# cvg/diffmvs

Measured on AMD Instinct MI355X. Metric: depth-maps/sec (640x512, 5 src views), higher is better.
Workload: dtype f32

## Files before the change

diffmvs_amd/_lib.py:

```python
from __future__ import annotations

import ctypes as C
import os

PKG = os.path.dirname(os.path.abspath(__file__))
HIP_LIB_PATH = os.environ.get("DMVS_LIB") or os.path.join(PKG, "libdmvs_hip.so")

ACT_NONE, ACT_RELU, ACT_SIGMOID, ACT_TANH, ACT_SILU = range(5)
IN_PLAIN, IN_UPSAMPLE2, IN_UNSHUFFLE2, IN_ZEROINSERT2 = range(4)
LAYOUT_NCHW, LAYOUT_NHWC, LAYOUT_NHWC_BF16, LAYOUT_NHWC_F16 = 0, 1, 2, 3
DTYPE_F32, DTYPE_BF16, DTYPE_F16, DTYPE_F32_PLAIN = 0, 1, 2, 3
ARITH_F32, ARITH_BF16, ARITH_SPLIT = 0, 1, 2
EW_DEPTH_TO_DISP, EW_DISP_TO_DEPTH = 0, 1

_P = C.c_void_p
_I = C.c_int32
_F = C.c_float


class Conv2dDesc(C.Structure):
    _fields_ = [
        ("in0", _P), ("in1", _P), ("mul0", _P), ("weight", _P), ("scale", _P), ("shift", _P),
        ("residual", _P), ("gru_z", _P), ("gru_h", _P), ("out", _P), ("gn_stats", _P), ("out_mul", _P),
        ("B", _I), ("c0", _I), ("c1", _I), ("Hin", _I), ("Win", _I), ("Hout", _I), ("Wout", _I),
# ... 18 lines not shown
        ("ref", _P), ("src", _P), ("rt", _P), ("inv_depth", _P), ("confidence", _P), ("view_w", _P),
        ("disp_min", _P), ("disp_max", _P), ("out_cost", _P), ("out_samples", _P), ("worklist", _P),
        ("B", _I), ("S", _I), ("C", _I), ("G", _I), ("n", _I), ("H", _I), ("W", _I), ("vw_shift", _I),
        ("cost_cstride", _I), ("cost_coffset", _I), ("samp_cstride", _I), ("samp_coffset", _I),
        ("interval", _F), ("min_radius", _F), ("max_radius", _F), ("feat_dtype", _I), ("tune", _I),
    ]


SIGNATURES = {
    "dmvs_abi_version": [],
    "dmvs_conv2d_f32": [C.POINTER(Conv2dDesc), _P],
    "dmvs_featurenet_stem_f32": [_P, _P, _P, _P, _P, _P, _P, _P, _I, _I, _I, _I, _P],
    "dmvs_featurenet_stem3_f32": [_P, _P, _P, _P, _P, _P, _P, _P, _P, _P, _P, _I, _I, _I, _I, _P],
    "dmvs_featurenet_conv1_pair_f32": [_P, _P, _P, _P, _P, _P, _P, _P, _I, _I, _I, _I, _P],
    "dmvs_featurenet_fpn_tail_f32": [_P, _P, _P, _P, _P, _P, _I, _I, _I, _I, _P],
    "dmvs_conv2d_wgrad_workspace_f32": [C.POINTER(Conv2dDesc), C.POINTER(C.c_int64)],
    "dmvs_conv2d_wgrad_f32": [C.POINTER(Conv2dDesc), _P, _P, _P, _P, C.c_int64, _P],
    "dmvs_conv3d_f32": [C.POINTER(Conv3dDesc), _P],
    "dmvs_conv3d_wgrad_workspace_f32": [C.POINTER(Conv3dDesc), C.POINTER(C.c_int64)],
    "dmvs_conv3d_wgrad_f32": [C.POINTER(Conv3dDesc), _P, _P, _P, _P, C.c_int64, _P],
    "dmvs_compose_proj_f32": [_P, _P, _I, _I, _P],
    "dmvs_warp_volume_f32": [_P, _P, _P, _P, _I, _I, _I, _I, _I, _I, _I, _P],
    "dmvs_getcost_quad_f32": [C.POINTER(GetCostDesc), _P],
    "dmvs_warp_corr_init_quad_f32": [_P, _P, _P, _P, _P, _P, _I, _I, _I, _I, _I, _I, _I, _I, _I, _I, _I, _P],
    "dmvs_warp_corr_init_bwd_f32": [_P, _P, _P, _P, _P, _P, _P, _P, _I, _I, _I, _I, _I, _I, _I, _I, _I, _I, _P],
    "dmvs_getcost_bwd_f32": [C.POINTER(GetCostDesc), _P, _P, _P, _P],
    "dmvs_view_aggregate_bwd_f32": [_P, _P, _P, _P, _P, _P, _I, _I, _I, _I, _P],
    "dmvs_view_aggregate_f32": [_P, _P, _P, _I, _I, _I, _I, _P],
    "dmvs_sigmoid_max_d_f32": [_P, _P, _I, _I, _I, _P],
    "dmvs_depth_regress_f32": [_P, _P, _P, _P, _P, _P, _I, _I, _I, _P],
# ... 38 lines not shown
VIEW_SELECT_MAX_IMAGES, VIEW_SELECT_MAX_LIST = 16384, 1 << 23
CLOUD_MAX_RINGS, CLOUD_MAX_KEY_BITS, CLOUD_MAX_THRESHOLDS = 1024, 62, 16
CLOUD_MOMENTS, CLOUD_MAX_POLYGON = 20, 256
DEPTH_MAX_THRESHOLDS, DEPTH_SLOTS = 8, 7
SPLAT_VIEW_CHUNK, SPLAT_VIEW_DOUBLES, SPLAT_SLOTS, SPLAT_MAX_RADIUS, SPLAT_NO_PRETEST = 8, 15, 4, 16, 0x1
NORMAL_MAX_RADIUS, NORMAL_CAM_DOUBLES, NORMAL_VIEW_CHUNK, NORMAL_SLOTS = 4, 27, 8, 4
TSDF_VIEW_CHUNK, TSDF_VIEW_DOUBLES, TSDF_MAX_VIEWS, TSDF_MAX_QUADS, TSDF_NO_CULL = 8, 12, 65535, 357913941, 0x1
RASTER_VIEW_DOUBLES, RASTER_SLOTS, RASTER_SMALL, RASTER_CULL_NEG, RASTER_CULL_POS = 22, 8, 64, 0x1, 0x2
ABI_VERSION = 4
TUNE_NO_WALK, TUNE_PIECES4, TUNE_NO_LEAN, TUNE_1X1_TILED, TUNE_NO_TALL, TUNE_TALL = 0x4, 0x8, 0x100, 0x200, 0x400, 0x800
TUNE3D_PIECES4, TUNE3D_S2_DIRECT, TUNE3D_NO_PAIR = 0x1, 0x2, 0x4
TUNE_SWEEP_GLOBAL = 0x1
TUNE_WGRAD_ACCUMULATE = 0x1000
TUNE_SPLIT_ALL = 0x20000
TUNE_STEM_EXACT = 0x40000


def tune_xcd_group(n: int) -> int:
    return (int(n) & 7) << 14


def tune3d_xcd_group(n: int) -> int:
    return (int(n) & 7) << 4
TUNE_BWD_INTERLEAVED, BWD_GATHER_INTERLEAVED = 0x1, 2


def tune_tile_wx(n: int) -> int:
    return n & 3


# ... 39 lines not shown
```

diffmvs_amd/csrc/conv1_pair.hip:

```cpp

#include "dmvs_common.h"
#include "dmvs_ring.h"
#include "dmvs_lds_poison.h"

namespace {

typedef float f32x4 __attribute__((ext_vector_type(4)));
typedef uint32_t u32x4s __attribute__((ext_vector_type(4)));

constexpr int PB = 512;
constexpr int US = 80, UR = 64;
constexpr int NP = US + 4;
typedef dmvs_ring<2, NP> Ring;
constexpr int PLQ = Ring::PLQ, RINGQ = Ring::RINGQ;
constexpr int NLOAD = 2 * 2 * NP;
constexpr int SW = US + 8;
constexpr int STAGEF = 2 * 16 * SW;
constexpr int NPIECE = STAGEF / 4;


__global__ void __launch_bounds__(PB) __attribute__((amdgpu_waves_per_eu(4, 4)))
featurenet_conv1_pair_kernel(const float* __restrict__ x, const u32x4s* __restrict__ ws1, const float* __restrict__ scale1,
                             const float* __restrict__ shift1, const u32x4s* __restrict__ ws2, const float* __restrict__ scale2,
                             const float* __restrict__ shift2, float* __restrict__ y, int N, int H, int W, int nsx, int nsy) {
    __shared__ __attribute__((aligned(16))) float lds[2 * RINGQ * 4 + STAGEF];
    DMVS_LDS_POISON(lds);

    const int tid = threadIdx.x, lane = tid & 63, wave = __builtin_amdgcn_readfirstlane(tid >> 6);
    const int m = lane & 15, kq = lane >> 4;
    const int role = wave >> 2, wr = wave & 3;
    const long plane = (long)H * W;
    const int iplane = H * W;
    const int nunits = nsx * nsy * N;

    const u32x4s* const wsp = role ? ws2 : ws1;
    u32x4s wq[2][3][3];
#pragma unroll
    for (int c = 0; c < 2; ++c)
#pragma unroll
        for (int g = 0; g < 3; ++g)
#pragma unroll
            for (int pl = 0; pl < 3; ++pl) wq[c][g][pl] = wsp[(((c * 3 + g) * 3 + pl) * 4 + kq) * 16 + m];
    const float* const scp = role ? scale2 : scale1;
    const float* const shp = role ? shift2 : shift1;
    const float sc = scp ? scp[m] : 1.0f, sh = shp ? shp[m] : 0.0f;
    int taps = 0;
#pragma unroll
    for (int g = 0; g < 3; ++g) taps |= dmvs_tap_slot<3, 3, 2>(g, kq) << (4 * g);
    const u32x4s* const src = reinterpret_cast<const u32x4s*>(lds) + role * RINGQ;
    u32x4s* const in_q = reinterpret_cast<u32x4s*>(lds);
    uint16_t* const mid_h = reinterpret_cast<uint16_t*>(lds) + RINGQ * 8;
    float* const stage = lds + 2 * RINGQ * 4;
    const int pmax = role ? US - 1 : US + 1;

    const int tb = tid - PB / 2;
    int lm = m, ltb = tb;

    for (int unit = blockIdx.x; unit < nunits; unit += gridDim.x) {
        const dmvs_unit u(unit, nsx, nsy, US, UR, H);
        const int n = u.n, X0 = u.X0, Y0 = u.Y0, Yend = u.Yend;
        const int nsteps = ((Yend - Y0 + 2) >> 1) + 4;
        const float* const xb = x + (long)n * 16 * plane;
        float* const yb = y + (long)n * 16 * plane;
        const int row_lo = role ? Y0 : max(Y0 - 1, 0), row_hi = role ? Yend : min(Yend + 1, H - 1);
        const int wlim = min(US, W - X0) + (role ? 0 : 2);
        auto conv_group = [&](int row, int cg) -> f32x4 {
            const int p = min(cg * 16 + lm, pmax);
            bf16x8 ph[2], pm, pl;
            auto qp_of = [&](int s) { return Ring::operand(s, taps, row, p); };
            {
                const int qp = qp_of(0);
                pl = __builtin_bit_cast(bf16x8, src[2 * PLQ + qp]);
                ph[0] = __builtin_bit_cast(bf16x8, src[qp]);
                pm = __builtin_bit_cast(bf16x8, src[PLQ + qp]);
            }
            f32x4 a = {0.0f, 0.0f, 0.0f, 0.0f};
// ... 125 lines not shown
                }
                DMVS_LDS_BARRIER();
            }
        }
    }
}

}

extern "C" int dmvs_featurenet_conv1_pair_f32(const float* x, const void* wsplit1, const float* scale1, const float* shift1, const void* wsplit2,
                                              const float* scale2, const float* shift2, float* y, int32_t N, int32_t H, int32_t W, int32_t tune,
                                              void* stream) {
    if (!x || !wsplit1 || !wsplit2 || !y || N <= 0 || H <= 0 || W <= 0) return DMVS_EINVAL;
    if ((long)16 * H * W >= (1L << 31)) return DMVS_EINVAL;
    if ((W & 3) || (((uintptr_t)x | (uintptr_t)y | (uintptr_t)wsplit1 | (uintptr_t)wsplit2) & 15)) return DMVS_EINVAL;
    const int nsx = (W + US - 1) / US, nsy = (H + UR - 1) / UR;
    const long nunits = (long)nsx * nsy * N;
    if (nunits >= (1L << 31)) return DMVS_EINVAL;
    static const int resident = dmvs_resident_workgroups(reinterpret_cast<const void*>(featurenet_conv1_pair_kernel), PB);
    hipLaunchKernelGGL(featurenet_conv1_pair_kernel, dim3(dmvs_persistent_grid(tune, resident, nunits)), dim3(PB), 0, (hipStream_t)stream, x,
                       reinterpret_cast<const u32x4s*>(wsplit1), scale1, shift1, reinterpret_cast<const u32x4s*>(wsplit2), scale2, shift2, y, N, H, W,
                       nsx, nsy);
    return dmvs_launch_status();
}
```

diffmvs_amd/csrc/dmvs_ring.h:

```cpp
#pragma once
#include "dmvs_bf16.h"

struct dmvs_unit {
    int sx, sy, n, X0, Y0, Yend;
    __device__ __forceinline__ dmvs_unit(int unit, int nsx, int nsy, int US, int UR, int H) {
        sx = unit % nsx;
        const int uq = unit / nsx;
        sy = uq % nsy;
        n = uq / nsy;
        X0 = US * sx;
        Y0 = UR * sy;
        Yend = min(Y0 + UR, H) - 1;
    }
};

template <int KH, int KW, int SH = 4> __device__ __forceinline__ int dmvs_tap_slot(int g, int kq) {
    const int t = min(4 * g + kq, KH * KW - 1);
    return (t / KW) | ((t % KW) << SH);
}

template <int NCH, int NP> struct dmvs_ring {
    static constexpr int SLOTS = 4;
    static constexpr int PLQ = SLOTS * NCH * NP;
    static constexpr int RINGQ = 3 * PLQ;
    static __device__ __forceinline__ int slot(int row) { return (row + 4) & 3; }
    static __device__ __forceinline__ int index(int row, int chunk, int pos) { return (slot(row) * NCH + chunk) * NP + pos; }
    static __device__ __forceinline__ int operand(int s, int taps, int row, int pos) {
        const int c = s / 3, g = s - c * 3;
        const int tg = taps >> (4 * g);
// ... 29 lines not shown
```

diffmvs_amd/csrc/fpn_tail.hip:

```cpp

#include "dmvs_common.h"
#include "dmvs_ring.h"
#include "dmvs_lds_poison.h"

namespace {

typedef float f32x4 __attribute__((ext_vector_type(4)));
typedef uint32_t u32x4s __attribute__((ext_vector_type(4)));

constexpr int PB = 256;
constexpr int US = 32, UR = 64;
constexpr int NP = US + 2;
constexpr int NCH = 8;
typedef dmvs_ring<NCH, NP> Ring;
constexpr int PLQ = Ring::PLQ, RINGQ = Ring::RINGQ;
constexpr int SW = US + 8;
constexpr int C2PIECE = 2 * 32 * SW / 4;
constexpr int CW = US / 2 + 8;
constexpr int C3PIECE = 64 * CW / 4;
constexpr int LDSF = RINGQ * 4 + C2PIECE * 4 + 2 * C3PIECE * 4;
constexpr int NSTEP = NCH * 3;

__global__ void __launch_bounds__(PB) __attribute__((amdgpu_waves_per_eu(2, 2)))
featurenet_fpn_tail_kernel(const float* __restrict__ c2, const float* __restrict__ c3, const float* __restrict__ w1, const float* __restrict__ b1,
                           const u32x4s* __restrict__ ws2, float* __restrict__ y, int N, int H, int W, int nsx, int nsy) {
    __shared__ __attribute__((aligned(16))) float lds[LDSF];
    DMVS_LDS_POISON(lds);

    const int tid = threadIdx.x, lane = tid & 63, wave = __builtin_amdgcn_readfirstlane(tid >> 6);
    const int m = lane & 15, kq = lane >> 4;
    const int H2 = H >> 1, W2 = W >> 1;
    const int iplane = H * W, iplane3 = H2 * W2;
    const int nunits = nsx * nsy * N;

    float w1r[8], b1r[4];
#pragma unroll
    for (int c = 0; c < 8; ++c) w1r[c] = w1[(4 * c + kq) * 64 + 16 * wave + m];
#pragma unroll
    for (int r = 0; r < 4; ++r) b1r[r] = b1 ? b1[16 * wave + 4 * kq + r] : 0.0f;
    const int nt = wave & 1, rr = wave >> 1;
    unsigned lwb = (unsigned)(kq * 32 + nt * 16 + m) * 16u;
    auto wload = [&](int sp) -> u32x4s {
        return *reinterpret_cast<const u32x4s*>(reinterpret_cast<const char*>(ws2 + sp * 128) + lwb);
    };
    int taps = 0;
#pragma unroll
    for (int g = 0; g < 3; ++g) taps |= dmvs_tap_slot<3, 3, 2>(g, kq) << (4 * g);
    u32x4s* const ring = reinterpret_cast<u32x4s*>(lds);
    float* const st2 = lds + RINGQ * 4;
    float* const st3 = st2 + C2PIECE * 4;

    int lm = m, ltid = tid;

    for (int unit = blockIdx.x; unit < nunits; unit += gridDim.x) {
        const dmvs_unit u(unit, nsx, nsy, US, UR, H);
        const int n = u.n, X0 = u.X0, Y0 = u.Y0, Yend = u.Yend;
        const int Q = (Yend - Y0 + 1) >> 1;
        const float* const c2b = c2 + (long)n * 32 * iplane;
        const float* const c3b = c3 + (long)n * 64 * iplane3;
        float* const yb = y + (long)n * 32 * iplane;

        auto stage_c3 = [&](int row3, int lt) {
#pragma unroll
            for (int k = 0; k < 2; ++k) {
                if (k * PB + wave * 64 < C3PIECE) {
                    const int e = k * PB + lt;
                    const int ch = e / (CW / 4), pc = e - ch * (CW / 4);
                    const int col = (X0 >> 1) - 4 + 4 * pc;
                    const bool ok = row3 >= 0 && row3 < H2 && col >= 0 && col < W2;
                    const float* srcp = ok ? c3b + (ch * iplane3 + row3 * W2 + col) : dmvs_zero16;
                    float* dstp = st3 + (((row3 + 2) & 1) * C3PIECE + k * PB + wave * 64) * 4;
                    __builtin_amdgcn_global_load_lds(srcp, DMVS_LDS_PTR(dstp), 16, 0, 0);
// ... 101 lines not shown
    }
}

}

extern "C" int dmvs_featurenet_fpn_tail_f32(const float* c2, const float* c3, const float* w_inner, const float* b_inner, const void* wsplit_out,
                                            float* y, int32_t N, int32_t H, int32_t W, int32_t tune, void* stream) {
    if (!c2 || !c3 || !w_inner || !wsplit_out || !y || N <= 0 || H <= 0 || W <= 0) return DMVS_EINVAL;
    if ((H & 1) || (W & 7) || (long)64 * H * W >= (1L << 31)) return DMVS_EINVAL;
    if ((((uintptr_t)c2 | (uintptr_t)c3 | (uintptr_t)y | (uintptr_t)wsplit_out) & 15) || ((uintptr_t)w_inner & 3) || ((uintptr_t)b_inner & 3))
        return DMVS_EINVAL;
    const int nsx = (W + US - 1) / US, nsy = (H + UR - 1) / UR;
    const long nunits = (long)nsx * nsy * N;
    if (nunits >= (1L << 31)) return DMVS_EINVAL;
    static const int resident = dmvs_resident_workgroups(reinterpret_cast<const void*>(featurenet_fpn_tail_kernel), PB);
    hipLaunchKernelGGL(featurenet_fpn_tail_kernel, dim3(dmvs_persistent_grid(tune, resident, nunits)), dim3(PB), 0, (hipStream_t)stream, c2, c3, w_inner, b_inner,
                       reinterpret_cast<const u32x4s*>(wsplit_out), y, N, H, W, nsx, nsy);
    return dmvs_launch_status();
}
```

diffmvs_amd/csrc/stem3.hip:

```cpp

#include "dmvs_common.h"
#include "dmvs_ring.h"
#include "dmvs_lds_poison.h"

#include <type_traits>

namespace {

typedef float f32x4 __attribute__((ext_vector_type(4)));
typedef uint32_t u32x4s __attribute__((ext_vector_type(4)));

constexpr int UC = 32, UR = 32;
constexpr int INW = 72;
constexpr int INROW = 3 * INW, INGRP = 4 * INROW;
constexpr int INSLOTS = 3;
constexpr int INF = INSLOTS * INGRP;
constexpr int NPIECE = INGRP / 4;
constexpr int MW = 2 * UC + 5, CW = 2 * UC + 3;
constexpr int MPL = 8 * MW, CPL = 8 * CW;
constexpr int MIDF = 3 * MPL * 4, C0F = 3 * CPL * 4;
constexpr int K0S = 9;
constexpr int K2S = 7;

__global__ void __launch_bounds__(DMVS_BLOCK) __attribute__((amdgpu_waves_per_eu(2, 2)))
featurenet_stem3_kernel(const float* __restrict__ x, const float* __restrict__ w0, const float* __restrict__ scale0, const float* __restrict__ shift0,
                        const float* __restrict__ w1, const float* __restrict__ scale1, const float* __restrict__ shift1,
                        const float* __restrict__ w2, const float* __restrict__ scale2, const float* __restrict__ shift2, float* __restrict__ y,
                        int N, int H, int W, int nsx, int nsy) {
    __shared__ __attribute__((aligned(16))) float lds[INF + MIDF + C0F];
    DMVS_LDS_POISON(lds);
    float* const s_in = lds;
    float* const s_mid = lds + INF;
    float* const s_c0 = s_mid + MIDF;

    const int tid = threadIdx.x, lane = tid & 63, wave = __builtin_amdgcn_readfirstlane(tid >> 6);
    const int m = lane & 15, kq = lane >> 4;
    const int Ho = H >> 1, Wo = W >> 1;
    const long plane = (long)H * W, oplane = (long)Ho * Wo;
    const int nunits = nsx * nsy * N;

    float a0[K0S];
    int koff[K0S];
#pragma unroll
    for (int s = 0; s < K0S; ++s) {
        const int k = 4 * s + kq;
        const int ci = k / 12, j = (k - ci * 12) / 3, kx = k % 3;
        const int ky = m < 8 ? j : j - 1;
        a0[s] = (ky >= 0 && ky <= 2) ? w0[(ci * 9 + ky * 3 + kx) * 8 + (m & 7)] : 0.0f;
        const int koff_a = j * INROW + ci * INW + kx;
        koff[s] = koff_a | ((koff_a + (j >= 2 ? 0 : 4 * INSLOTS * INROW)) << 16);
    }
    float sc0[4], sh0[4], sc1[4], sh1[4];
#pragma unroll
    for (int r = 0; r < 4; ++r) {
// ... 12 lines not shown
    int off2[K2S];
#pragma unroll
    for (int s = 0; s < K2S; ++s) {
        const int sl = 4 * s + kq;
        float wv[8];
#pragma unroll
        for (int ci = 0; ci < 8; ++ci) wv[ci] = sl < 25 ? w2[(ci * 25 + sl) * 16 + m] : 0.0f;
        dmvs_split3_bf16x8(wv, w2h[s], w2m[s], w2l[s]);
        off2[s] = dmvs_tap_slot<5, 5>(s, kq);
    }
    const float sc2 = scale2 ? scale2[m] : 1.0f, sh2 = shift2 ? shift2[m] : 0.0f;
    const bool vec = (Wo & 3) == 0 && ((uintptr_t)y & 15) == 0;

    const int p_i = tid / (NPIECE / 4), p_rem = tid - p_i * (NPIECE / 4);
    const int p_ci = p_rem / (INW / 4), p_c = (p_rem - p_ci * (INW / 4)) * 4;
    auto stage = [&](int unit, int kg, int slot) {
        const dmvs_unit u(unit, nsx, nsy, UC, UR, Ho);
        const int row = 2 * u.Y0 - 5 + 4 * kg + p_i, col = 2 * u.X0 - 4 + p_c;
        if (tid < NPIECE) {
            const bool ok = row >= 0 && row < H && col >= 0 && col < W;
            const float* srcp = ok ? x + ((long)u.n * 3 + p_ci) * plane + (long)row * W + col : dmvs_zero16;
            float* dstp = s_in + slot * INGRP + wave * 256;
            __builtin_amdgcn_global_load_lds(srcp, DMVS_LDS_PTR(dstp), 16, 0, 0);
        }
    };

    auto steps_of = [&](int unit) {
        const dmvs_unit u(unit, nsx, nsy, UC, UR, Ho);
        return ((u.Yend - u.Y0 + 2) >> 1) + 2;
    };
    int s_unit = blockIdx.x, s_k = 0, s_slot = 0, s_steps = s_unit < nunits ? steps_of(s_unit) : 0;
    auto stage_next = [&]() {
        if (s_unit < nunits) {
            stage(s_unit, s_k, s_slot);
            s_slot = s_slot == INSLOTS - 1 ? 0 : s_slot + 1;
            if (++s_k == s_steps) {
                s_unit += gridDim.x;
                s_k = 0;
                s_steps = s_unit < nunits ? steps_of(s_unit) : 0;
            }
        }
    };
    int islot = 0, pslot = INSLOTS - 1;
    int unit = blockIdx.x;
    stage_next();
    stage_next();
    DMVS_DMA_BARRIER();
    for (; unit < nunits; unit += gridDim.x) {
        const dmvs_unit u(unit, nsx, nsy, UC, UR, Ho);
        const int n = u.n, ox0 = u.X0, oy0 = u.Y0, X0 = 2 * ox0, Y0 = 2 * oy0;
        const int nsteps = steps_of(unit);
        for (int k = 0; k < nsteps; ++k, pslot = islot, islot = islot == INSLOTS - 1 ? 0 : islot + 1) {
            {
                const int sbeg = k == 0 ? MW : 0;
                const int ng = (2 * MW - sbeg + 15) >> 4;
                auto conv00 = [&](auto ngc, int g0) {
                    constexpr int NG = decltype(ngc)::value;
                    int q[NG], pm[NG];
                    float b[NG][K0S];
                    f32x4 acc[NG];
#pragma unroll
                    for (int i = 0; i < NG; ++i) {
                        const int p = min(sbeg + (g0 + 4 * i) * 16 + m, 2 * MW - 1);
                        q[i] = p >= MW ? 1 : 0;
                        pm[i] = p - q[i] * MW;
                        const int rb = q[i] ? 4 * islot : 4 * pslot + 2;
// ... 92 lines not shown
#pragma unroll
                        for (int r = 0; r < 4; ++r)
                            if (ox + r < Wo) dst[r] = v[r];
                    }
                }
            }
        }
    }
}

}

extern "C" int dmvs_featurenet_stem3_f32(const float* x, const float* w0, const float* scale0, const float* shift0, const float* w1,
                                         const float* scale1, const float* shift1, const float* w2, const float* scale2, const float* shift2,
                                         float* y, int32_t N, int32_t H, int32_t W, int32_t tune, void* stream) {
    (void)tune;
    if (!x || !w0 || !w1 || !w2 || !y || N <= 0 || H <= 0 || W <= 0) return DMVS_EINVAL;
    if ((long)3 * H * W >= (1L << 31)) return DMVS_EINVAL;
    if ((H & 1) || (W & 3) || ((uintptr_t)x & 15)) return DMVS_EINVAL;
    const int nsx = (W / 2 + UC - 1) / UC, nsy = (H / 2 + UR - 1) / UR;
    const long nunits = (long)nsx * nsy * N;
    if (nunits >= (1L << 31)) return DMVS_EINVAL;
    static const int resident = dmvs_resident_workgroups(reinterpret_cast<const void*>(featurenet_stem3_kernel));
    const unsigned grid = (unsigned)(nunits < resident ? nunits : resident);
    hipLaunchKernelGGL(featurenet_stem3_kernel, dim3(grid), dim3(DMVS_BLOCK), 0, (hipStream_t)stream, x, w0, scale0, shift0, w1, scale1, shift1, w2,
                       scale2, shift2, y, N, H, W, nsx, nsy);
    return dmvs_launch_status();
}
```

diffmvs_amd/ops.py:

```python
from __future__ import annotations

import ctypes as C
import os
from dataclasses import dataclass
from typing import Optional

import torch

from . import _lib
from ._lib import (ACT_NONE, ACT_RELU, ACT_SIGMOID, ACT_SILU, ACT_TANH, ARITH_BF16, ARITH_F32, ARITH_SPLIT, DTYPE_BF16, DTYPE_F16, DTYPE_F32, IN_PLAIN,
                   IN_UNSHUFFLE2, IN_UPSAMPLE2, IN_ZEROINSERT2, LAYOUT_NCHW, LAYOUT_NHWC, LAYOUT_NHWC_BF16, LAYOUT_NHWC_F16)

CONV_ARITH = {"fp32": ARITH_F32, "bf16": ARITH_BF16, "split": ARITH_SPLIT}
FEATURE_DTYPES = {"fp32": torch.float32, "bf16": torch.bfloat16, "fp16": torch.float16}
_DTYPE_CODE = {torch.float32: DTYPE_F32, torch.bfloat16: DTYPE_BF16, torch.float16: DTYPE_F16}
_NHWC_LAYOUT = {torch.float32: LAYOUT_NHWC, torch.bfloat16: LAYOUT_NHWC_BF16, torch.float16: LAYOUT_NHWC_F16}


def _round_up(x: int, m: int) -> int:
    return (x + m - 1) // m * m


@dataclass
class PackedConv:
# ... 117 lines not shown
def _env_tune():
    e = os.environ.get
    t2 = _lib.tune_tile_wx(int(e("DMVS_CONV_WX", "0"))) | _lib.tune_tile_mt(int(e("DMVS_CONV_MT", "0")))
    t2 |= _lib.TUNE_NO_WALK if e("DMVS_CONV_WALK") == "0" else 0
    t2 |= _lib.TUNE_PIECES4 if e("DMVS_CONV_V16") == "0" else 0
    t2 |= _lib.TUNE_NO_LEAN if e("DMVS_CONV_LEAN") == "0" else 0
    t2 |= _lib.TUNE_1X1_TILED if e("DMVS_CONV1X1_PX4") == "0" else 0
    t2 |= {"0": _lib.TUNE_NO_TALL, "1": _lib.TUNE_TALL}.get(e("DMVS_CONV_TALL"), 0)
    t2 |= _lib.TUNE_SPLIT_ALL if e("DMVS_CONV_SPLIT_ALL") == "1" else 0
    t2 |= _lib.tune_xcd_group(int(e("DMVS_CONV_XCD", "0")))
    t3 = (_lib.TUNE3D_PIECES4 if e("DMVS_CONV3D_V16") == "0" else 0) | (_lib.TUNE3D_S2_DIRECT if e("DMVS_CONV3D_S2") == "direct" else 0)
    t3 |= _lib.TUNE3D_NO_PAIR if e("DMVS_CONV3D_PAIR") == "0" else 0
    t3 |= _lib.tune3d_xcd_group(int(e("DMVS_CONV3D_XCD", "0")))
    return {"conv2d": t2, "conv3d": t3, "stem": (_lib.TUNE_PIECES4 if e("DMVS_STEM_V16") == "0" else 0) | _lib.tune_xcd_group(int(e("DMVS_STEM_XCD", "0"))) | (_lib.TUNE_STEM_EXACT if e("DMVS_STEM_EXACT") == "1" else 0),
            "sweep": _lib.TUNE_SWEEP_GLOBAL if e("DMVS_PLANE_SWEEP") == "quad" else 0,
            "bwd_gather": e("DMVS_GETCOST_BWD") == "gather",
            "bwd_il": e("DMVS_BWD_INTERLEAVED", "%d" % BWD_INTERLEAVED_DEFAULT) == "1"}


class Ops:
    _bindings = {}

    def __init__(self, lib: _lib.Lib, device):
        self.lib = lib
        self.device = torch.device(device)
        self.tune = _env_tune()
        self.timers = None
        self.conv_arith = ARITH_F32
        self.debug_fill = None
        self.getcost_hook = None
# ... 144 lines not shown
        self._stem_launch(pc0, pc1, x, y, tune)
        return y

    def _stem_launch(self, pc0: PackedConv, pc1: PackedConv, x, y, tune=None):
        N, cin, H, W = x.shape
        if not (cin == 3 and pc0.cin == 3 and pc0.cout == 8 and pc1.cin == 8 and pc1.cout == 8 and pc0.k == (3, 3) and
                pc1.k == (3, 3) and pc0.stride == 1 and pc1.stride == 1 and pc0.pad == (1, 1) and pc1.pad == (1, 1) and
                pc0.cout_pad == 8 and pc1.cout_pad == 8):
            raise _lib.DmvsError("featurenet_stem: expects the 3->8->8 3x3 stem of FeatureNet")
        tune = self.tune["stem"] if tune is None else tune
        if self.conv_arith != ARITH_SPLIT:
            tune |= _lib.TUNE_STEM_EXACT
        self._call("dmvs_featurenet_stem_f32", _ptr(x), _ptr(pc0.weight), _ptr(pc0.scale), _ptr(pc0.shift), _ptr(pc1.weight),
                   _ptr(pc1.scale), _ptr(pc1.shift), _ptr(y), N, H, W, tune, self.stream())

    @staticmethod
    def featurenet_stem3_supported(x):
        xs = x if isinstance(x, (list, tuple)) else [x]
        H, W = xs[0].shape[2], xs[0].shape[3]
        return H % 2 == 0 and W % 4 == 0 and 3 * H * W < 2 ** 31 and all(t.data_ptr() % 16 == 0 for t in xs)

    def featurenet_stem3(self, pc0: PackedConv, pc1: PackedConv, pc2: PackedConv, x, tune=None):
        xs = x if isinstance(x, (list, tuple)) else [x]
        self._chk(*xs)
        Bv, cin, H, W = xs[0].shape
        if not (cin == 3 and pc0.cin == 3 and pc0.cout == 8 and pc1.cin == 8 and pc1.cout == 8 and pc0.k == (3, 3) and
                pc1.k == (3, 3) and pc0.stride == 1 and pc1.stride == 1 and pc0.pad == (1, 1) and pc1.pad == (1, 1) and
                pc0.cout_pad == 8 and pc1.cout_pad == 8 and pc2.cin == 8 and pc2.cout == 16 and pc2.cout_pad == 16 and pc2.k == (5, 5) and
                pc2.stride == 2 and pc2.pad == (2, 2)):
            raise _lib.DmvsError("featurenet_stem3: expects the 3->8->8 3x3 stem of FeatureNet and its 8->16 5x5 stride-2 conv1.0")
        if not self.featurenet_stem3_supported(xs) or any(t.shape != xs[0].shape for t in xs):
            raise _lib.DmvsError(f"featurenet_stem3: needs even H, W % 4 == 0 and 16-byte aligned views of one shape, got {tuple(xs[0].shape)}")
        y = self.empty(len(xs) * Bv, 16, H // 2, W // 2)
        for v, xv in enumerate(xs):
            self._call("dmvs_featurenet_stem3_f32", _ptr(xv), _ptr(pc0.weight), _ptr(pc0.scale), _ptr(pc0.shift), _ptr(pc1.weight),
                       _ptr(pc1.scale), _ptr(pc1.shift), _ptr(pc2.weight), _ptr(pc2.scale), _ptr(pc2.shift), _ptr(y[v * Bv:(v + 1) * Bv]),
                       Bv, H, W, 0 if tune is None else tune, self.stream())
        return y

    CONV1_PAIR_STRIP, CONV1_PAIR_SEGMENT = 80, 64

    @staticmethod
    def conv1_pair_supported(x):
        return (x.dim() == 4 and x.shape[1] == 16 and x.shape[3] % 4 == 0 and 16 * x.shape[2] * x.shape[3] < 2 ** 31 and
                x.data_ptr() % 16 == 0)

    def conv1_pair(self, pc1: PackedConv, pc2: PackedConv, x, tune=0):
        self._chk(x)
        for pc in (pc1, pc2):
            if not (pc.cin == 16 and pc.cout == 16 and pc.cout_pad == 16 and pc.k == (3, 3) and pc.stride == 1 and pc.pad == (1, 1)):
                raise _lib.DmvsError("conv1_pair: expects the two 16->16 3x3 stride-1 layers of FeatureNet's conv1")
        if not self.conv1_pair_supported(x):
            raise _lib.DmvsError(f"conv1_pair: needs 16 channels, W % 4 == 0 and a 16-byte aligned tensor, got {tuple(x.shape)}")
        N, _, H, W = x.shape
        y = self.empty(N, 16, H, W)
        self._call("dmvs_featurenet_conv1_pair_f32", _ptr(x), _ptr(split_weights(pc1)), _ptr(pc1.scale), _ptr(pc1.shift),
                   _ptr(split_weights(pc2)), _ptr(pc2.scale), _ptr(pc2.shift), _ptr(y), N, H, W, tune, self.stream())
        return y

    FPN_TAIL_STRIP, FPN_TAIL_SEGMENT = 32, 64

    @staticmethod
    def fpn_tail_supported(c2, c3):
        if not (c2.dim() == 4 and c3.dim() == 4 and c2.dtype == torch.float32 and c3.dtype == torch.float32):
            return False
        N, C, H, W = c2.shape
        return (C == 32 and H % 2 == 0 and W % 8 == 0 and H > 0 and W > 0 and tuple(c3.shape) == (N, 64, H // 2, W // 2) and
                64 * H * W < 2 ** 31 and c2.is_contiguous() and c3.is_contiguous() and c2.data_ptr() % 16 == 0 and c3.data_ptr() % 16 == 0)

    def fpn_tail(self, pc_inner: PackedConv, pc_out: PackedConv, c2, c3, tune=0):
        self._chk(c2, c3)
        if not (pc_inner.cin == 32 and pc_inner.cout == 64 and pc_inner.cout_pad == 64 and pc_inner.k == (1, 1) and pc_inner.stride == 1 and
                pc_inner.pad == (0, 0) and pc_inner.scale is None and pc_out.cin == 64 and pc_out.cout == 32 and pc_out.cout_pad == 32 and
                pc_out.k == (3, 3) and pc_out.stride == 1 and pc_out.pad == (1, 1) and pc_out.scale is None and pc_out.shift is None):
            raise _lib.DmvsError("fpn_tail: expects FeatureNet's inner1 (32->64 1x1, bias) and out2 (64->32 3x3, no bias)")
        if not self.fpn_tail_supported(c2, c3):
            raise _lib.DmvsError(f"fpn_tail: needs c2 [N,32,H,W] and c3 [N,64,H/2,W/2] with even H, W % 8 == 0, contiguous and 16-byte aligned, "
                                 f"got {tuple(c2.shape)} and {tuple(c3.shape)}")
        N, _, H, W = c2.shape
        y = self.empty(N, H, W, 32)
        self._call("dmvs_featurenet_fpn_tail_f32", _ptr(c2), _ptr(c3), _ptr(pc_inner.weight), _ptr(pc_inner.shift), _ptr(split_weights(pc_out)),
                   _ptr(y), N, H, W, tune, self.stream())
        return y

    def conv2d_wgrad(self, pc: PackedConv, x0, grad_out, x1=None, *, mul0=None, in_mode=IN_PLAIN, want_bias=False, tune=None,
                     into_gw=None, into_gb=None):
        self._chk(x0, x1, mul0, grad_out, into_gw, into_gb)
        B = x0.shape[0]
        if in_mode == IN_PLAIN:
            c0, Hin, Win = x0.shape[1], x0.shape[2], x0.shape[3]
        elif in_mode in (IN_UPSAMPLE2, IN_ZEROINSERT2):
            c0, Hin, Win = x0.shape[1], x0.shape[2] * 2, x0.shape[3] * 2
        else:
            c0, Hin, Win = x0.shape[1] * 4, x0.shape[2] // 2, x0.shape[3] // 2
        c1 = 0 if x1 is None else x1.shape[1]
        kh, kw = pc.k
        Hout, Wout = grad_out.shape[2], grad_out.shape[3]
# ... 681 lines not shown
```

include/dmvs.h:

```cpp
#ifndef DMVS_H
#define DMVS_H

#include <stdint.h>

#ifdef __cplusplus
extern "C" {
#endif

#define DMVS_ABI_VERSION 4
#define DMVS_EINVAL (-22)

enum { DMVS_ACT_NONE = 0, DMVS_ACT_RELU = 1, DMVS_ACT_SIGMOID = 2, DMVS_ACT_TANH = 3, DMVS_ACT_SILU = 4 };
enum { DMVS_IN_PLAIN = 0, DMVS_IN_UPSAMPLE2 = 1 , DMVS_IN_UNSHUFFLE2 = 2 ,
       DMVS_IN_ZEROINSERT2 = 3  };
enum { DMVS_LAYOUT_NCHW = 0, DMVS_LAYOUT_NHWC = 1,
       DMVS_LAYOUT_NHWC_BF16 = 2, DMVS_LAYOUT_NHWC_F16 = 3 };
enum { DMVS_DTYPE_F32 = 0 , DMVS_DTYPE_BF16 = 1, DMVS_DTYPE_F16 = 2 ,
       DMVS_DTYPE_F32_PLAIN = 3  };

int dmvs_abi_version(void);

#define DMVS_ARITH_F32 0
#define DMVS_ARITH_BF16 1
#define DMVS_ARITH_SPLIT 2
// ... 35 lines not shown
    float post_scale;
    int32_t gate_cstride;
    int32_t arith;
    int32_t tune;
    int32_t out_mul_c0;
    int32_t in0_cstride;
    const void* weight_split;
} dmvs_conv2d_desc;

int dmvs_conv2d_f32(const dmvs_conv2d_desc* d, void* stream);

int dmvs_featurenet_stem_f32(const float* x, const float* w0, const float* scale0, const float* shift0, const float* w1,
                             const float* scale1, const float* shift1, float* y, int32_t N, int32_t H, int32_t W, int32_t tune,
                             void* stream);

int dmvs_featurenet_stem3_f32(const float* x, const float* w0, const float* scale0, const float* shift0, const float* w1,
                              const float* scale1, const float* shift1, const float* w2, const float* scale2, const float* shift2,
                              float* y, int32_t N, int32_t H, int32_t W, int32_t tune, void* stream);

int dmvs_featurenet_conv1_pair_f32(const float* x, const void* wsplit1, const float* scale1, const float* shift1, const void* wsplit2,
                                   const float* scale2, const float* shift2, float* y, int32_t N, int32_t H, int32_t W, int32_t tune,
                                   void* stream);

int dmvs_featurenet_fpn_tail_f32(const float* c2, const float* c3, const float* w_inner, const float* b_inner, const void* wsplit_out,
                                 float* y, int32_t N, int32_t H, int32_t W, int32_t tune, void* stream);

#define DMVS_TUNE_WGRAD_ACCUMULATE 0x1000
int dmvs_conv2d_wgrad_workspace_f32(const dmvs_conv2d_desc* d, int64_t* bytes);
int dmvs_conv2d_wgrad_f32(const dmvs_conv2d_desc* d, const float* grad_out, float* gw, float* gb, float* workspace,
                          int64_t workspace_bytes, void* stream);

typedef struct dmvs_conv3d_desc {
    const float* in;
    const float* weight;
    const float* scale;
    const float* shift;
    const float* residual;
    float* out;
    int32_t B, cin, cout, cout_pad;
    int32_t Din, Hin, Win;
// ... 224 lines not shown
```

Baseline: 1499.

## Balance persistent featurenet kernels by splitting row work into contiguous spans

Replaces the fixed 64-row segment work units in the stem3, conv1_pair and fpn_tail persistent kernels with a march scheme. Each workgroup gets a contiguous, nearly equal span of row-pairs across columns and images, with boundaries snapped to pieces of at least 8 pairs. This is meant to remove tail imbalance when the number of units does not divide evenly over resident workgroups, and to reduce the halo re-priming that happens at each segment start. Spans are on by default for stem3 and conv1_pair and off for fpn_tail, with env/tune flags to override. The cost is that spans crossing image or column boundaries add prologue restarts, and the grid size changes.

New measurement: 1513 (median of 6 runs). Within noise of the previous version (+0.9%).

```diff
diff --git a/diffmvs_amd/_lib.py b/diffmvs_amd/_lib.py
--- a/diffmvs_amd/_lib.py
+++ b/diffmvs_amd/_lib.py
@@ -56,6 +56,7 @@
     "dmvs_featurenet_stem3_f32": [_P, _P, _P, _P, _P, _P, _P, _P, _P, _P, _P, _I, _I, _I, _I, _P],
     "dmvs_featurenet_conv1_pair_f32": [_P, _P, _P, _P, _P, _P, _P, _P, _I, _I, _I, _I, _P],
     "dmvs_featurenet_fpn_tail_f32": [_P, _P, _P, _P, _P, _P, _I, _I, _I, _I, _P],
+    "dmvs_march_span_pieces": [_I, _I, _I, _I, _P, _I, _P, _P],
     "dmvs_conv2d_wgrad_workspace_f32": [C.POINTER(Conv2dDesc), C.POINTER(C.c_int64)],
     "dmvs_conv2d_wgrad_f32": [C.POINTER(Conv2dDesc), _P, _P, _P, _P, C.c_int64, _P],
     "dmvs_conv3d_f32": [C.POINTER(Conv3dDesc), _P],
@@ -124,6 +125,7 @@
 TUNE_WGRAD_ACCUMULATE = 0x1000
 TUNE_SPLIT_ALL = 0x20000
 TUNE_STEM_EXACT = 0x40000
+TUNE_FIXED_SEGMENTS, TUNE_MARCH_SPANS = 0x100000, 0x200000
 
 
 def tune_xcd_group(n: int) -> int:
diff --git a/diffmvs_amd/csrc/conv1_pair.hip b/diffmvs_amd/csrc/conv1_pair.hip
--- a/diffmvs_amd/csrc/conv1_pair.hip
+++ b/diffmvs_amd/csrc/conv1_pair.hip
@@ -10,6 +10,7 @@
 
 constexpr int PB = 512;
 constexpr int US = 80, UR = 64;
+constexpr bool SPANS_DEFAULT = true;
 constexpr int NP = US + 4;
 typedef dmvs_ring<2, NP> Ring;
 constexpr int PLQ = Ring::PLQ, RINGQ = Ring::RINGQ;
@@ -22,7 +23,7 @@
 __global__ void __launch_bounds__(PB) __attribute__((amdgpu_waves_per_eu(4, 4)))
 featurenet_conv1_pair_kernel(const float* __restrict__ x, const u32x4s* __restrict__ ws1, const float* __restrict__ scale1,
                              const float* __restrict__ shift1, const u32x4s* __restrict__ ws2, const float* __restrict__ scale2,
-                             const float* __restrict__ shift2, float* __restrict__ y, int N, int H, int W, int nsx, int nsy) {
+                             const float* __restrict__ shift2, float* __restrict__ y, int N, int H, int W, int nsx, int P, int UP) {
     __shared__ __attribute__((aligned(16))) float lds[2 * RINGQ * 4 + STAGEF];
     DMVS_LDS_POISON(lds);
 
@@ -31,7 +32,6 @@
     const int role = wave >> 2, wr = wave & 3;
     const long plane = (long)H * W;
     const int iplane = H * W;
-    const int nunits = nsx * nsy * N;
 
     const u32x4s* const wsp = role ? ws2 : ws1;
     u32x4s wq[2][3][3];
@@ -56,10 +56,9 @@
     const int tb = tid - PB / 2;
     int lm = m, ltb = tb;
 
-    for (int unit = blockIdx.x; unit < nunits; unit += gridDim.x) {
-        const dmvs_unit u(unit, nsx, nsy, US, UR, H);
-        const int n = u.n, X0 = u.X0, Y0 = u.Y0, Yend = u.Yend;
-        const int nsteps = ((Yend - Y0 + 2) >> 1) + 4;
+    for (dmvs_march walk(blockIdx.x, gridDim.x, N, nsx, P, UP); walk.next();) {
+        const int n = walk.n, X0 = US * walk.sx, Y0 = 2 * walk.p0, Yend = min(2 * walk.p1, H) - 1;
+        const int nsteps = walk.p1 - walk.p0 + 4;
         const float* const xb = x + (long)n * 16 * plane;
         float* const yb = y + (long)n * 16 * plane;
         const int row_lo = role ? Y0 : max(Y0 - 1, 0), row_hi = role ? Yend : min(Yend + 1, H - 1);
@@ -215,12 +214,13 @@
     if (!x || !wsplit1 || !wsplit2 || !y || N <= 0 || H <= 0 || W <= 0) return DMVS_EINVAL;
     if ((long)16 * H * W >= (1L << 31)) return DMVS_EINVAL;
     if ((W & 3) || (((uintptr_t)x | (uintptr_t)y | (uintptr_t)wsplit1 | (uintptr_t)wsplit2) & 15)) return DMVS_EINVAL;
-    const int nsx = (W + US - 1) / US, nsy = (H + UR - 1) / UR;
+    const int nsx = (W + US - 1) / US, nsy = (H + UR - 1) / UR, P = (H + 1) / 2;
     const long nunits = (long)nsx * nsy * N;
     if (nunits >= (1L << 31)) return DMVS_EINVAL;
     static const int resident = dmvs_resident_workgroups(reinterpret_cast<const void*>(featurenet_conv1_pair_kernel), PB);
-    hipLaunchKernelGGL(featurenet_conv1_pair_kernel, dim3(dmvs_persistent_grid(tune, resident, nunits)), dim3(PB), 0, (hipStream_t)stream, x,
+    const dmvs_march_launch plan = dmvs_march_plan(tune, resident, (long)nsx * N, P, UR / 2, SPANS_DEFAULT);
+    hipLaunchKernelGGL(featurenet_conv1_pair_kernel, dim3(plan.grid), dim3(PB), 0, (hipStream_t)stream, x,
                        reinterpret_cast<const u32x4s*>(wsplit1), scale1, shift1, reinterpret_cast<const u32x4s*>(wsplit2), scale2, shift2, y, N, H, W,
-                       nsx, nsy);
+                       nsx, P, plan.up);
     return dmvs_launch_status();
 }
diff --git a/diffmvs_amd/csrc/dmvs_ring.h b/diffmvs_amd/csrc/dmvs_ring.h
--- a/diffmvs_amd/csrc/dmvs_ring.h
+++ b/diffmvs_amd/csrc/dmvs_ring.h
@@ -1,18 +1,66 @@
 #pragma once
 #include "dmvs_bf16.h"
 
-struct dmvs_unit {
-    int sx, sy, n, X0, Y0, Yend;
-    __device__ __forceinline__ dmvs_unit(int unit, int nsx, int nsy, int US, int UR, int H) {
-        sx = unit % nsx;
-        const int uq = unit / nsx;
-        sy = uq % nsy;
-        n = uq / nsy;
-        X0 = US * sx;
-        Y0 = UR * sy;
-        Yend = min(Y0 + UR, H) - 1;
+#define DMVS_SPAN_PIECE 8
+#define DMVS_SPAN_MIN (2 * DMVS_SPAN_PIECE)
+#if defined(__HIP_DEVICE_COMPILE__) && !defined(DMVS_HOST_EMULATION)
+#define DMVS_UNIFORM(v) __builtin_amdgcn_readfirstlane(v)
+#else
+#define DMVS_UNIFORM(v) (v)
+#endif
+
+__host__ __device__ __forceinline__ int dmvs_span_bound(int g, int G, int T, int P) {
+    const int q = T / G, rem = T - q * G;
+    int b = g * q + (int)((unsigned)g * (unsigned)rem / (unsigned)G);
+    const int r = b % P;
+    if (P < 2 * DMVS_SPAN_PIECE)
+        b += 2 * r < P ? -r : P - r;
+    else if (r < DMVS_SPAN_PIECE)
+        b -= r;
+    else if (P - r < DMVS_SPAN_PIECE)
+        b -= DMVS_SPAN_PIECE - (P - r);
+    return DMVS_UNIFORM(b);
+}
+
+struct dmvs_march {
+    int nsx, P, UP, nsy;
+    int pos, end, stride;
+    int n, sx, p0, p1;
+    __host__ __device__ __forceinline__ dmvs_march(int g, int G, int N, int nsx_, int P_, int UP_) : nsx(nsx_), P(P_), UP(UP_) {
+        n = sx = p0 = p1 = 0;
+        const int up = UP ? UP : P;
+        nsy = DMVS_UNIFORM((P + up - 1) / up);
+        const int T = (int)((unsigned)N * (unsigned)nsx * (unsigned)P);
+        const int b0 = dmvs_span_bound(g, G, T, P), b1 = dmvs_span_bound(g + 1, G, T, P);
+        pos = UP ? g : b0;
+        end = UP ? nsx * nsy * N : b1;
+        stride = UP ? G : 0;
+    }
+    __host__ __device__ __forceinline__ bool next() {
+        if (pos >= end) return false;
+        const int d0 = UP ? nsx : P, q0 = DMVS_UNIFORM(pos / d0), r0 = pos - q0 * d0;
+        const int d1 = UP ? nsy : nsx, q1 = DMVS_UNIFORM(q0 / d1), r1 = q0 - q1 * d1;
+        n = q1;
+        sx = UP ? r0 : r1;
+        p0 = UP ? UP * r1 : r0;
+        const int len = UP ? UP : end - pos;
+        p1 = p0 + len < P ? p0 + len : P;
+        pos += UP ? stride : p1 - p0;
+        return true;
     }
 };
+
+struct dmvs_march_launch {
+    unsigned grid;
+    int up;
+};
+static inline dmvs_march_launch dmvs_march_plan(int tune, int resident, long ncols, int P, int UP, bool spans_default) {
+    const long T = ncols * P;
+    const bool spans = T < (1L << 31) && ((tune & DMVS_TUNE_MARCH_SPANS) || (spans_default && !(tune & DMVS_TUNE_FIXED_SEGMENTS)));
+    if (!spans) return {dmvs_persistent_grid(tune, resident, ncols * ((P + UP - 1) / UP)), UP};
+    const long most = T / DMVS_SPAN_MIN > 1 ? T / DMVS_SPAN_MIN : 1;
+    return {dmvs_persistent_grid(tune, resident, most), 0};
+}
 
 template <int KH, int KW, int SH = 4> __device__ __forceinline__ int dmvs_tap_slot(int g, int kq) {
     const int t = min(4 * g + kq, KH * KW - 1);
diff --git a/diffmvs_amd/csrc/fpn_tail.hip b/diffmvs_amd/csrc/fpn_tail.hip
--- a/diffmvs_amd/csrc/fpn_tail.hip
+++ b/diffmvs_amd/csrc/fpn_tail.hip
@@ -10,6 +10,7 @@
 
 constexpr int PB = 256;
 constexpr int US = 32, UR = 64;
+constexpr bool SPANS_DEFAULT = false;
 constexpr int NP = US + 2;
 constexpr int NCH = 8;
 typedef dmvs_ring<NCH, NP> Ring;
@@ -23,7 +24,7 @@
 
 __global__ void __launch_bounds__(PB) __attribute__((amdgpu_waves_per_eu(2, 2)))
 featurenet_fpn_tail_kernel(const float* __restrict__ c2, const float* __restrict__ c3, const float* __restrict__ w1, const float* __restrict__ b1,
-                           const u32x4s* __restrict__ ws2, float* __restrict__ y, int N, int H, int W, int nsx, int nsy) {
+                           const u32x4s* __restrict__ ws2, float* __restrict__ y, int N, int H, int W, int nsx, int P, int UP) {
     __shared__ __attribute__((aligned(16))) float lds[LDSF];
     DMVS_LDS_POISON(lds);
 
@@ -31,7 +32,6 @@
     const int m = lane & 15, kq = lane >> 4;
     const int H2 = H >> 1, W2 = W >> 1;
     const int iplane = H * W, iplane3 = H2 * W2;
-    const int nunits = nsx * nsy * N;
 
     float w1r[8], b1r[4];
 #pragma unroll
@@ -52,10 +52,9 @@
 
     int lm = m, ltid = tid;
 
-    for (int unit = blockIdx.x; unit < nunits; unit += gridDim.x) {
-        const dmvs_unit u(unit, nsx, nsy, US, UR, H);
-        const int n = u.n, X0 = u.X0, Y0 = u.Y0, Yend = u.Yend;
-        const int Q = (Yend - Y0 + 1) >> 1;
+    for (dmvs_march walk(blockIdx.x, gridDim.x, N, nsx, P, UP); walk.next();) {
+        const int n = walk.n, X0 = US * walk.sx, Y0 = 2 * walk.p0;
+        const int Q = walk.p1 - walk.p0;
         const float* const c2b = c2 + (long)n * 32 * iplane;
         const float* const c3b = c3 + (long)n * 64 * iplane3;
         float* const yb = y + (long)n * 32 * iplane;
@@ -187,7 +186,8 @@
     const long nunits = (long)nsx * nsy * N;
     if (nunits >= (1L << 31)) return DMVS_EINVAL;
     static const int resident = dmvs_resident_workgroups(reinterpret_cast<const void*>(featurenet_fpn_tail_kernel), PB);
-    hipLaunchKernelGGL(featurenet_fpn_tail_kernel, dim3(dmvs_persistent_grid(tune, resident, nunits)), dim3(PB), 0, (hipStream_t)stream, c2, c3, w_inner, b_inner,
-                       reinterpret_cast<const u32x4s*>(wsplit_out), y, N, H, W, nsx, nsy);
+    const dmvs_march_launch plan = dmvs_march_plan(tune, resident, (long)nsx * N, H / 2, UR / 2, SPANS_DEFAULT);
+    hipLaunchKernelGGL(featurenet_fpn_tail_kernel, dim3(plan.grid), dim3(PB), 0, (hipStream_t)stream, c2, c3, w_inner, b_inner,
+                       reinterpret_cast<const u32x4s*>(wsplit_out), y, N, H, W, nsx, H / 2, plan.up);
     return dmvs_launch_status();
 }
diff --git a/diffmvs_amd/csrc/stem3.hip b/diffmvs_amd/csrc/stem3.hip
--- a/diffmvs_amd/csrc/stem3.hip
+++ b/diffmvs_amd/csrc/stem3.hip
@@ -11,6 +11,7 @@
 typedef uint32_t u32x4s __attribute__((ext_vector_type(4)));
 
 constexpr int UC = 32, UR = 32;
+constexpr bool SPANS_DEFAULT = true;
 constexpr int INW = 72;
 constexpr int INROW = 3 * INW, INGRP = 4 * INROW;
 constexpr int INSLOTS = 3;
@@ -26,7 +27,7 @@
 featurenet_stem3_kernel(const float* __restrict__ x, const float* __restrict__ w0, const float* __restrict__ scale0, const float* __restrict__ shift0,
                         const float* __restrict__ w1, const float* __restrict__ scale1, const float* __restrict__ shift1,
                         const float* __restrict__ w2, const float* __restrict__ scale2, const float* __restrict__ shift2, float* __restrict__ y,
-                        int N, int H, int W, int nsx, int nsy) {
+                        int N, int H, int W, int nsx, int P, int UP) {
     __shared__ __attribute__((aligned(16))) float lds[INF + MIDF + C0F];
     DMVS_LDS_POISON(lds);
     float* const s_in = lds;
@@ -37,7 +38,6 @@
     const int m = lane & 15, kq = lane >> 4;
     const int Ho = H >> 1, Wo = W >> 1;
     const long plane = (long)H * W, oplane = (long)Ho * Wo;
-    const int nunits = nsx * nsy * N;
 
     float a0[K0S];
     int koff[K0S];
@@ -80,42 +80,37 @@
 
     const int p_i = tid / (NPIECE / 4), p_rem = tid - p_i * (NPIECE / 4);
     const int p_ci = p_rem / (INW / 4), p_c = (p_rem - p_ci * (INW / 4)) * 4;
-    auto stage = [&](int unit, int kg, int slot) {
-        const dmvs_unit u(unit, nsx, nsy, UC, UR, Ho);
-        const int row = 2 * u.Y0 - 5 + 4 * kg + p_i, col = 2 * u.X0 - 4 + p_c;
+    auto stage = [&](const dmvs_march& w, int kg, int slot) {
+        const int row = 4 * w.p0 - 5 + 4 * kg + p_i, col = 2 * UC * w.sx - 4 + p_c;
         if (tid < NPIECE) {
             const bool ok = row >= 0 && row < H && col >= 0 && col < W;
-            const float* srcp = ok ? x + ((long)u.n * 3 + p_ci) * plane + (long)row * W + col : dmvs_zero16;
+            const float* srcp = ok ? x + ((long)w.n * 3 + p_ci) * plane + (long)row * W + col : dmvs_zero16;
             float* dstp = s_in + slot * INGRP + wave * 256;
             __builtin_amdgcn_global_load_lds(srcp, DMVS_LDS_PTR(dstp), 16, 0, 0);
         }
     };
 
-    auto steps_of = [&](int unit) {
-        const dmvs_unit u(unit, nsx, nsy, UC, UR, Ho);
-        return ((u.Yend - u.Y0 + 2) >> 1) + 2;
-    };
-    int s_unit = blockIdx.x, s_k = 0, s_slot = 0, s_steps = s_unit < nunits ? steps_of(s_unit) : 0;
+    dmvs_march walk(blockIdx.x, gridDim.x, N, nsx, P, UP);
+    dmvs_march ahead = walk;
+    bool s_more = ahead.next();
+    int s_k = 0, s_slot = 0;
     auto stage_next = [&]() {
-        if (s_unit < nunits) {
-            stage(s_unit, s_k, s_slot);
+        if (s_more) {
+            stage(ahead, s_k, s_slot);
             s_slot = s_slot == INSLOTS - 1 ? 0 : s_slot + 1;
-            if (++s_k == s_steps) {
-                s_unit += gridDim.x;
+            if (++s_k == ahead.p1 - ahead.p0 + 2) {
+                s_more = ahead.next();
                 s_k = 0;
-                s_steps = s_unit < nunits ? steps_of(s_unit) : 0;
             }
         }
     };
     int islot = 0, pslot = INSLOTS - 1;
-    int unit = blockIdx.x;
     stage_next();
     stage_next();
     DMVS_DMA_BARRIER();
-    for (; unit < nunits; unit += gridDim.x) {
-        const dmvs_unit u(unit, nsx, nsy, UC, UR, Ho);
-        const int n = u.n, ox0 = u.X0, oy0 = u.Y0, X0 = 2 * ox0, Y0 = 2 * oy0;
-        const int nsteps = steps_of(unit);
+    while (walk.next()) {
+        const int n = walk.n, ox0 = UC * walk.sx, oy0 = 2 * walk.p0, X0 = 2 * ox0, Y0 = 2 * oy0;
+        const int nsteps = walk.p1 - walk.p0 + 2;
         for (int k = 0; k < nsteps; ++k, pslot = islot, islot = islot == INSLOTS - 1 ? 0 : islot + 1) {
             {
                 const int sbeg = k == 0 ? MW : 0;
@@ -238,16 +233,32 @@
 extern "C" int dmvs_featurenet_stem3_f32(const float* x, const float* w0, const float* scale0, const float* shift0, const float* w1,
                                          const float* scale1, const float* shift1, const float* w2, const float* scale2, const float* shift2,
                                          float* y, int32_t N, int32_t H, int32_t W, int32_t tune, void* stream) {
-    (void)tune;
     if (!x || !w0 || !w1 || !w2 || !y || N <= 0 || H <= 0 || W <= 0) return DMVS_EINVAL;
     if ((long)3 * H * W >= (1L << 31)) return DMVS_EINVAL;
     if ((H & 1) || (W & 3) || ((uintptr_t)x & 15)) return DMVS_EINVAL;
-    const int nsx = (W / 2 + UC - 1) / UC, nsy = (H / 2 + UR - 1) / UR;
+    const int nsx = (W / 2 + UC - 1) / UC, nsy = (H / 2 + UR - 1) / UR, P = (H / 2 + 1) / 2;
     const long nunits = (long)nsx * nsy * N;
     if (nunits >= (1L << 31)) return DMVS_EINVAL;
     static const int resident = dmvs_resident_workgroups(reinterpret_cast<const void*>(featurenet_stem3_kernel));
-    const unsigned grid = (unsigned)(nunits < resident ? nunits : resident);
-    hipLaunchKernelGGL(featurenet_stem3_kernel, dim3(grid), dim3(DMVS_BLOCK), 0, (hipStream_t)stream, x, w0, scale0, shift0, w1, scale1, shift1, w2,
-                       scale2, shift2, y, N, H, W, nsx, nsy);
+    const dmvs_march_launch plan = dmvs_march_plan(tune, resident, (long)nsx * N, P, UR / 2, SPANS_DEFAULT);
+    hipLaunchKernelGGL(featurenet_stem3_kernel, dim3(plan.grid), dim3(DMVS_BLOCK), 0, (hipStream_t)stream, x, w0, scale0, shift0, w1, scale1, shift1, w2,
+                       scale2, shift2, y, N, H, W, nsx, P, plan.up);
     return dmvs_launch_status();
 }
+
+extern "C" int dmvs_march_span_pieces(int32_t N, int32_t nsx, int32_t P, int32_t G, int32_t* pieces, int32_t capacity, int32_t* count, int32_t* grid) {
+    if (N <= 0 || nsx <= 0 || P <= 0 || G <= 0 || G > 0xffff || capacity < 0 || !pieces || !count || !grid) return DMVS_EINVAL;
+    if ((long)N * nsx * P >= (1L << 31)) return DMVS_EINVAL;
+    const dmvs_march_launch plan = dmvs_march_plan(G | DMVS_TUNE_MARCH_SPANS, G, (long)N * nsx, P, 1, true);
+    int32_t k = 0;
+    for (int g = 0; g < (int)plan.grid; ++g) {
+        for (dmvs_march walk(g, (int)plan.grid, N, nsx, P, 0); walk.next(); ++k) {
+            if (k >= capacity) return DMVS_EINVAL;
+            const int32_t row[5] = {g, walk.n, walk.sx, walk.p0, walk.p1};
+            for (int i = 0; i < 5; ++i) pieces[5 * k + i] = row[i];
+        }
+    }
+    count[0] = k;
+    grid[0] = (int32_t)plan.grid;
+    return 0;
+}
diff --git a/diffmvs_amd/ops.py b/diffmvs_amd/ops.py
--- a/diffmvs_amd/ops.py
+++ b/diffmvs_amd/ops.py
@@ -155,6 +155,7 @@
     t3 |= _lib.tune3d_xcd_group(int(e("DMVS_CONV3D_XCD", "0")))
     return {"conv2d": t2, "conv3d": t3, "stem": (_lib.TUNE_PIECES4 if e("DMVS_STEM_V16") == "0" else 0) | _lib.tune_xcd_group(int(e("DMVS_STEM_XCD", "0"))) | (_lib.TUNE_STEM_EXACT if e("DMVS_STEM_EXACT") == "1" else 0),
             "sweep": _lib.TUNE_SWEEP_GLOBAL if e("DMVS_PLANE_SWEEP") == "quad" else 0,
+            "march": {"0": _lib.TUNE_FIXED_SEGMENTS, "1": _lib.TUNE_MARCH_SPANS}.get(e("DMVS_MARCH_SPANS"), 0),
             "bwd_gather": e("DMVS_GETCOST_BWD") == "gather",
             "bwd_il": e("DMVS_BWD_INTERLEAVED", "%d" % BWD_INTERLEAVED_DEFAULT) == "1"}
 
@@ -329,6 +330,10 @@
         self._call("dmvs_featurenet_stem_f32", _ptr(x), _ptr(pc0.weight), _ptr(pc0.scale), _ptr(pc0.shift), _ptr(pc1.weight),
                    _ptr(pc1.scale), _ptr(pc1.shift), _ptr(y), N, H, W, tune, self.stream())
 
+    def _march_tune(self, tune):
+        t = tune or 0
+        return t if t & (_lib.TUNE_FIXED_SEGMENTS | _lib.TUNE_MARCH_SPANS) else t | self.tune["march"]
+
     @staticmethod
     def featurenet_stem3_supported(x):
         xs = x if isinstance(x, (list, tuple)) else [x]
@@ -350,7 +355,7 @@
         for v, xv in enumerate(xs):
             self._call("dmvs_featurenet_stem3_f32", _ptr(xv), _ptr(pc0.weight), _ptr(pc0.scale), _ptr(pc0.shift), _ptr(pc1.weight),
                        _ptr(pc1.scale), _ptr(pc1.shift), _ptr(pc2.weight), _ptr(pc2.scale), _ptr(pc2.shift), _ptr(y[v * Bv:(v + 1) * Bv]),
-                       Bv, H, W, 0 if tune is None else tune, self.stream())
+                       Bv, H, W, self._march_tune(tune), self.stream())
         return y
 
     CONV1_PAIR_STRIP, CONV1_PAIR_SEGMENT = 80, 64
@@ -360,7 +365,7 @@
         return (x.dim() == 4 and x.shape[1] == 16 and x.shape[3] % 4 == 0 and 16 * x.shape[2] * x.shape[3] < 2 ** 31 and
                 x.data_ptr() % 16 == 0)
 
-    def conv1_pair(self, pc1: PackedConv, pc2: PackedConv, x, tune=0):
+    def conv1_pair(self, pc1: PackedConv, pc2: PackedConv, x, tune=None):
         self._chk(x)
         for pc in (pc1, pc2):
             if not (pc.cin == 16 and pc.cout == 16 and pc.cout_pad == 16 and pc.k == (3, 3) and pc.stride == 1 and pc.pad == (1, 1)):
@@ -370,7 +375,8 @@
         N, _, H, W = x.shape
         y = self.empty(N, 16, H, W)
         self._call("dmvs_featurenet_conv1_pair_f32", _ptr(x), _ptr(split_weights(pc1)), _ptr(pc1.scale), _ptr(pc1.shift),
-                   _ptr(split_weights(pc2)), _ptr(pc2.scale), _ptr(pc2.shift), _ptr(y), N, H, W, tune, self.stream())
+                   _ptr(split_weights(pc2)), _ptr(pc2.scale), _ptr(pc2.shift), _ptr(y), N, H, W,
+                   self._march_tune(tune), self.stream())
         return y
 
     FPN_TAIL_STRIP, FPN_TAIL_SEGMENT = 32, 64
@@ -383,7 +389,7 @@
         return (C == 32 and H % 2 == 0 and W % 8 == 0 and H > 0 and W > 0 and tuple(c3.shape) == (N, 64, H // 2, W // 2) and
                 64 * H * W < 2 ** 31 and c2.is_contiguous() and c3.is_contiguous() and c2.data_ptr() % 16 == 0 and c3.data_ptr() % 16 == 0)
 
-    def fpn_tail(self, pc_inner: PackedConv, pc_out: PackedConv, c2, c3, tune=0):
+    def fpn_tail(self, pc_inner: PackedConv, pc_out: PackedConv, c2, c3, tune=None):
         self._chk(c2, c3)
         if not (pc_inner.cin == 32 and pc_inner.cout == 64 and pc_inner.cout_pad == 64 and pc_inner.k == (1, 1) and pc_inner.stride == 1 and
                 pc_inner.pad == (0, 0) and pc_inner.scale is None and pc_out.cin == 64 and pc_out.cout == 32 and pc_out.cout_pad == 32 and
@@ -395,7 +401,7 @@
         N, _, H, W = c2.shape
         y = self.empty(N, H, W, 32)
         self._call("dmvs_featurenet_fpn_tail_f32", _ptr(c2), _ptr(c3), _ptr(pc_inner.weight), _ptr(pc_inner.shift), _ptr(split_weights(pc_out)),
-                   _ptr(y), N, H, W, tune, self.stream())
+                   _ptr(y), N, H, W, self._march_tune(tune), self.stream())
         return y
 
     def conv2d_wgrad(self, pc: PackedConv, x0, grad_out, x1=None, *, mul0=None, in_mode=IN_PLAIN, want_bias=False, tune=None,
diff --git a/include/dmvs.h b/include/dmvs.h
--- a/include/dmvs.h
+++ b/include/dmvs.h
@@ -73,6 +73,8 @@
                              const float* scale1, const float* shift1, float* y, int32_t N, int32_t H, int32_t W, int32_t tune,
                              void* stream);
 
+#define DMVS_TUNE_FIXED_SEGMENTS 0x100000
+#define DMVS_TUNE_MARCH_SPANS 0x200000
 int dmvs_featurenet_stem3_f32(const float* x, const float* w0, const float* scale0, const float* shift0, const float* w1,
                               const float* scale1, const float* shift1, const float* w2, const float* scale2, const float* shift2,
                               float* y, int32_t N, int32_t H, int32_t W, int32_t tune, void* stream);
@@ -83,6 +85,8 @@
 
 int dmvs_featurenet_fpn_tail_f32(const float* c2, const float* c3, const float* w_inner, const float* b_inner, const void* wsplit_out,
                                  float* y, int32_t N, int32_t H, int32_t W, int32_t tune, void* stream);
+
+int dmvs_march_span_pieces(int32_t N, int32_t nsx, int32_t P, int32_t G, int32_t* pieces, int32_t capacity, int32_t* count, int32_t* grid);
 
 #define DMVS_TUNE_WGRAD_ACCUMULATE 0x1000
 int dmvs_conv2d_wgrad_workspace_f32(const dmvs_conv2d_desc* d, int64_t* bytes);
```
